# alibaba/unified-audio

Measured on AMD Instinct MI355X. Metric: audio-seconds/sec H-Codec encode+decode @16kHz b=32, higher is better.
Workload: dtype f32

## Files before the change

include/quarkaudio.h:

```cpp
#ifndef QUARKAUDIO_H_
#define QUARKAUDIO_H_

#include <stdint.h>

#ifdef __cplusplus
extern "C" {
#endif

#define QA_VERSION 103

typedef enum qa_status {
    QA_OK = 0,
    QA_ERR_INVALID = -1,
    QA_ERR_HIP = -2,
    QA_ERR_MISSING = -3,
    QA_ERR_UNSUPPORTED = -4
} qa_status;

typedef struct qa_tensor {
    const char* name;
    const float* data;
    int64_t numel;
} qa_tensor;

// ... 114 lines not shown
    int32_t post_act;
    int32_t in_rep;
} qa_conv_args;
int qa_conv1d_cl(const qa_conv_args* args, void* stream);

int qa_weight_planes(const float* w, int64_t n, void* planes, void* stream);
int qa_weight_planes_attach(const float* w, int64_t n, const void* planes);
int qa_weight_planes_detach(const float* w);
int64_t qa_weight_planes_bytes(void);
int64_t qa_weight_plane_offset(int64_t index, int32_t plane);

int qa_sconv_geometry(int64_t L, int32_t ksize, int32_t stride, int64_t* T_out, int32_t* pad_left, int32_t* pad_right);
int64_t qa_resolve_frame(int64_t r, int64_t L, int32_t max_pad, int32_t pad_mode);

int qa_profile_begin(void);
int qa_profile_end(double* out, int32_t n_out);
int qa_profile_begin_ex(int32_t mask);
int qa_profile_hbm_kinds(void);
const char* qa_profile_hbm_name(int32_t kind);
int qa_profile_end_hbm(double* out, int32_t n_out);
int qa_set_serial(int32_t on);

int qa_debug_lstm_stats(int32_t device, int64_t* out4);

int qa_knob_count(void);
int qa_knob_info(int32_t index, const char** name, int64_t* value, int64_t* default_value, const char** doc);
int qa_set_knob(const char* name, int64_t value);
int qa_get_knob(const char* name, int64_t* value);

typedef struct qa_ssl_spec {
    int32_t n_conv;
    int32_t conv_dim[8];
    int32_t conv_kernel[8];
    int32_t conv_stride[8];
    int32_t conv_bias;
    int32_t feat_norm_layer;
    int32_t hidden;
    int32_t n_layers;
    int32_t n_heads;
    int32_t intermediate;
    int32_t stable_layer_norm;
    int32_t pos_kernel;
    int32_t pos_groups;
    int32_t pad;
    int32_t n_select;
    int32_t select[32];
// ... 184 lines not shown
```

unified_audio_amd/_lib.py:

```python
from __future__ import annotations

import ctypes as C
import os
from typing import Optional

_HERE = os.path.dirname(os.path.abspath(__file__))
_LIB_NAME = "libquarkaudio_hip.so"
_lib: Optional[C.CDLL] = None


class QuarkAudioError(RuntimeError):

    def __init__(self, status: int, message: str):
        super().__init__(f"[qa_status {status}] {message}")
        self.status = status


class qa_tensor(C.Structure):
    _fields_ = [("name", C.c_char_p), ("data", C.c_void_p), ("numel", C.c_int64)]


class qa_hcodec_spec(C.Structure):
    _fields_ = [
        ("n_filters", C.c_int32), ("n_ratios", C.c_int32), ("ratios", C.c_int32 * 8), ("dimension", C.c_int32),
# ... 111 lines not shown
    "qa_hcodec_forward_adaptive": (C.c_int, [C.c_void_p, C.c_void_p, C.c_int64, C.c_int64, C.c_void_p, C.c_int64, C.c_int64,
                                             C.c_int64, C.c_int64, C.c_void_p, C.c_void_p, C.c_void_p, C.POINTER(C.c_int64),
                                             C.c_void_p]),
    "qa_hcodec_enable_taps": (C.c_int, [C.c_void_p, C.c_int]),
    "qa_hcodec_tap": (C.c_int64, [C.c_void_p, C.c_char_p, C.c_void_p, C.c_int64, C.c_void_p]),
    "qa_rvq_search": (C.c_int, [C.c_void_p, C.c_int64, C.c_void_p, C.c_int32, C.c_int32, C.c_int32, C.c_void_p,
                                C.c_void_p, C.c_void_p]),
    "qa_rvq_lookup": (C.c_int, [C.c_void_p, C.c_int64, C.c_void_p, C.c_int32, C.c_int32, C.c_int32, C.c_void_p,
                                C.c_void_p]),
    "qa_conv1d_cl": (C.c_int, [C.POINTER(qa_conv_args), C.c_void_p]),
    "qa_weight_planes": (C.c_int, [C.c_void_p, C.c_int64, C.c_void_p, C.c_void_p]),
    "qa_weight_planes_attach": (C.c_int, [C.c_void_p, C.c_int64, C.c_void_p]),
    "qa_weight_planes_detach": (C.c_int, [C.c_void_p]),
    "qa_weight_planes_bytes": (C.c_int64, []),
    "qa_weight_plane_offset": (C.c_int64, [C.c_int64, C.c_int32]),
    "qa_sconv_geometry": (C.c_int, [C.c_int64, C.c_int32, C.c_int32, C.POINTER(C.c_int64), C.POINTER(C.c_int32), C.POINTER(C.c_int32)]),
    "qa_resolve_frame": (C.c_int64, [C.c_int64, C.c_int64, C.c_int32, C.c_int32]),
    "qa_profile_begin": (C.c_int, []),
    "qa_profile_end": (C.c_int, [C.POINTER(C.c_double), C.c_int32]),
    "qa_profile_begin_ex": (C.c_int, [C.c_int32]),
    "qa_profile_hbm_kinds": (C.c_int, []),
    "qa_profile_hbm_name": (C.c_char_p, [C.c_int32]),
    "qa_debug_lstm_stats": (C.c_int, [C.c_int32, C.POINTER(C.c_int64)]),
    "qa_profile_end_hbm": (C.c_int, [C.POINTER(C.c_double), C.c_int32]),
    "qa_set_serial": (C.c_int, [C.c_int32]),
    "qa_knob_count": (C.c_int, []),
    "qa_knob_info": (C.c_int, [C.c_int32, C.POINTER(C.c_char_p), C.POINTER(C.c_int64), C.POINTER(C.c_int64), C.POINTER(C.c_char_p)]),
    "qa_set_knob": (C.c_int, [C.c_char_p, C.c_int64]),
    "qa_get_knob": (C.c_int, [C.c_char_p, C.POINTER(C.c_int64)]),
    "qa_mimi_create": (C.c_int, [C.POINTER(C.c_void_p), C.POINTER(qa_mimi_spec), C.POINTER(qa_tensor), C.c_int64, C.c_char_p, C.c_int]),
    "qa_mimi_destroy": (None, [C.c_void_p]),
    "qa_mimi_forward": (C.c_int, [C.c_void_p, C.c_void_p, C.c_int64, C.c_int64, C.c_void_p, C.c_void_p]),
    "qa_mimi_stream_begin": (C.c_int, [C.c_void_p, C.c_int64]),
    "qa_mimi_stream_step": (C.c_int, [C.c_void_p, C.c_void_p, C.c_int64, C.c_void_p, C.c_void_p]),
    "qa_mimi_stream_reset": (C.c_int, [C.c_void_p]),
    "qa_mimi_stream_end": (C.c_int, [C.c_void_p]),
    "qa_mimi_stream_offset": (C.c_int64, [C.c_void_p]),
    "qa_ssl_create": (C.c_int, [C.POINTER(C.c_void_p), C.POINTER(qa_ssl_spec), C.POINTER(qa_tensor), C.c_int64, C.c_int]),
    "qa_ssl_destroy": (None, [C.c_void_p]),
    "qa_ssl_frames": (C.c_int64, [C.c_void_p, C.c_int64]),
    "qa_ssl_forward": (C.c_int, [C.c_void_p, C.c_void_p, C.c_int64, C.c_int64, C.c_void_p, C.c_void_p]),
    "qa_bicodec_create": (C.c_int, [C.POINTER(C.c_void_p), C.POINTER(qa_bicodec_spec), C.POINTER(qa_tensor), C.c_int64, C.c_int]),
    "qa_bicodec_destroy": (None, [C.c_void_p]),
    "qa_bicodec_hop": (C.c_int64, [C.c_void_p]),
    "qa_bicodec_detokenize": (C.c_int, [C.c_void_p, C.c_void_p, C.c_void_p, C.c_int64, C.c_int64, C.c_void_p, C.c_void_p]),
    "qa_bicodec_enable_taps": (C.c_int, [C.c_void_p, C.c_int]),
# ... 119 lines not shown
```

unified_audio_amd/csrc/attention.hip:

```cpp
#include "kernels.h"

#ifdef QA_ATT_TIMING
__device__ unsigned long long g_qa_att_timing[8];
#define QA_ATT_TICK(i)                                      \
    {                                                       \
        const long long now_ = __builtin_readcyclecounter(); \
        tacc[i] += now_ - tlast;                            \
        tlast = now_;                                       \
    }
extern "C" int qa_debug_att_timing(unsigned long long* out, int reset) {
    if (out && hipMemcpyFromSymbol(out, HIP_SYMBOL(g_qa_att_timing), sizeof(g_qa_att_timing)) != hipSuccess) return -1;
    if (reset) {
        unsigned long long z[8] = {0};
        if (hipMemcpyToSymbol(HIP_SYMBOL(g_qa_att_timing), z, sizeof(z)) != hipSuccess) return -1;
    }
    return 0;
}
#else
#define QA_ATT_TICK(i)
#endif

namespace qa {

typedef float f32x16 __attribute__((ext_vector_type(16)));
// ... 183 lines not shown
    if (lane == 0) {
        for (int i = 0; i < 4; ++i) atomicAdd(&g_qa_att_timing[i], (unsigned long long)tacc[i]);
        atomicAdd(&g_qa_att_timing[4], (unsigned long long)(tlast - tbegin));
        atomicAdd(&g_qa_att_timing[5], 1ULL);
        atomicAdd(&g_qa_att_timing[6], (unsigned long long)n_done);
    }
#endif

    if (qi < n_q) {
        const float inv = l_run > 0.f ? 1.f / l_run : 0.f;
        float* op = out + ((long long)b * n_q + qi) * ldo + head * HD + 4 * hh;
#pragma unroll
        for (int t = 0; t < DT; ++t)
#pragma unroll
            for (int c = 0; c < 4; ++c) {
                float4 w;
                w.x = o[t][4 * c + 0] * inv; w.y = o[t][4 * c + 1] * inv;
                w.z = o[t][4 * c + 2] * inv; w.w = o[t][4 * c + 3] * inv;
                *reinterpret_cast<float4*>(op + 32 * t + 8 * c) = w;
            }
    }
}

int launch_attention(const float* q, long long ldq, const float* k, const float* v, long long ldkv, float* out,
                     long long ldo, int B, int n_q, int n_keys, long long kv_batch_stride, int H, int hd, float scale,
                     int causal, hipStream_t s, const float* gate, const float* relbias, int R, int context, int q_pos0,
                     int ring_end, const unsigned char* kvalid) {
    QA_REQUIRE(n_q > 0 && n_keys > 0 && (!causal || ring_end > 0 || n_keys >= n_q), "attention: n_q=%d n_keys=%d", n_q, n_keys);
    QA_REQUIRE(context >= 0 && (context == 0 || causal) && (ring_end <= 0 || (causal && context > 0 && !gate)),
               "attention: a context window needs causal=1; the ring mode needs causal=1 and context > 0");
    QA_REQUIRE((ldq % 4) == 0 && (ldkv % 4) == 0 && (ldo % 4) == 0, "attention: strides must be multiples of 4");
    QA_REQUIRE((gate == nullptr) == (relbias == nullptr) && (!gate || (R >= 0 && !causal && n_q == n_keys)),
               "attention: gate and relbias come together, for non-causal self-attention");
    QA_REQUIRE(!kvalid || (!gate && !causal && n_q == n_keys), "attention: the key-padding mask is for non-causal self-attention without bias");
    dim3 grid((unsigned)ceil_div(n_q, 128), H, B);
    const int dbg = (int)knob(K_ATT_DEBUG);
#define QA_ATT(HD)                                                                                                          \
    if (kvalid)                                                                                                              \
        hipLaunchKernelGGL((attention_kernel<HD, false, true>), grid, dim3(256), 0, s, q, ldq, k, v, ldkv, kv_batch_stride, out, ldo, n_q, \
                           n_keys, scale, causal, nullptr, nullptr, 0, context, q_pos0, ring_end, dbg, kvalid);                 \
    else if (gate)                                                                                                                \
        hipLaunchKernelGGL((attention_kernel<HD, true>), grid, dim3(256), 0, s, q, ldq, k, v, ldkv, kv_batch_stride, out, ldo, n_q, \
                           n_keys, scale, causal, gate, relbias, R, context, q_pos0, ring_end, dbg, nullptr);                           \
    else                                                                                                                     \
        hipLaunchKernelGGL((attention_kernel<HD, false>), grid, dim3(256), 0, s, q, ldq, k, v, ldkv, kv_batch_stride, out, ldo, n_q, \
                           n_keys, scale, causal, nullptr, nullptr, 0, context, q_pos0, ring_end, dbg, nullptr)
    switch (hd) {
        case 32: QA_ATT(32); break;
        case 64: QA_ATT(64); break;
        case 96: QA_ATT(96); break;
        case 128: QA_ATT(128); break;
        default: qa::set_error("attention: head_dim=%d unsupported (32/64/96/128)", hd); return QA_ERR_UNSUPPORTED;
    }
#undef QA_ATT
    QA_LAUNCH_CHECK();
    return QA_OK;
}

}

extern "C" int qa_debug_attention(const float* q, long long ldq, const float* k, const float* v, long long ldkv, float* out, long long ldo,
                                  int B, int n_q, int n_keys, long long kv_bstride, int H, int hd, float scale, int causal, void* stream) {
    return qa::launch_attention(q, ldq, k, v, ldkv, out, ldo, B, n_q, n_keys, kv_bstride, H, hd, scale, causal,
                                static_cast<hipStream_t>(stream));
}

extern "C" int qa_debug_attention_ex(const float* q, long long ldq, const float* k, const float* v, long long ldkv, float* out,
                                     long long ldo, int B, int n_q, int n_keys, long long kv_bstride, int H, int hd, float scale,
                                     int causal, const float* gate, const float* relbias, int R, int context, int q_pos0, int ring_end,
                                     void* stream) {
    return qa::launch_attention(q, ldq, k, v, ldkv, out, ldo, B, n_q, n_keys, kv_bstride, H, hd, scale, causal,
                                static_cast<hipStream_t>(stream), gate, relbias, R, context, q_pos0, ring_end);
}
```

unified_audio_amd/csrc/host_util.h:

```cpp
#pragma once
#include <algorithm>
#include <cmath>
#include <cstring>
#include <string>
#include <unordered_map>
#include <utility>
#include <vector>

#include "kernels.h"
#include "split_planes.h"

namespace qa {

class HostTable {
   public:
    HostTable(const qa_tensor* t, int64_t n) {
        for (int64_t i = 0; i < n; ++i)
            if (t[i].name && t[i].data) map_[t[i].name] = &t[i];
    }
    const float* get(const std::string& name, int64_t numel) const {
        auto it = map_.find(name);
        if (it == map_.end()) {
            set_error("weight table: missing tensor '%s'", name.c_str());
            return nullptr;
// ... 98 lines not shown
    }
    int ensure(size_t bytes) {
        if (bytes <= cap) return QA_OK;
        if (ptr) QA_HIP(hipFree(ptr));
        ptr = nullptr;
        cap = 0;
        const size_t grown = bytes + bytes / 8;
        QA_HIP(hipMalloc(reinterpret_cast<void**>(&ptr), grown));
        cap = grown;
        return QA_OK;
    }
};

struct Tap {
    const float* ptr;
    int64_t numel;
};

struct Ctx {
    Arena arena;
    hipStream_t stream = nullptr;
    bool dry = false;
    bool gemm_fp32 = false;
    bool capture = false;
    std::unordered_map<std::string, Tap> taps;
    void tap(const std::string& name, const float* p, int64_t n) {
        if (!capture) return;
        float* copy = arena.alloc<float>((size_t)n);
        arena.pin();
        if (dry) return;
        (void)hipMemcpyAsync(copy, p, sizeof(float) * (size_t)n, hipMemcpyDeviceToDevice, stream);
        taps[name] = Tap{copy, n};
    }
};

struct ConvW {
    const float* w = nullptr;
    const float* b = nullptr;
    int N = 0, C_in = 0, ksize = 1;
    int algo_n = 0, algo_cin = 0;
};

inline int pad32(int c) { return (int)round_up(c, 32); }


enum { WN_NONE = 0, WN_FOLD = 1, WN_DETECT = 2 };
// ... 143 lines not shown
inline int layernorm_op(Ctx& c, const float* x, const float* w, const float* b, float* y, int64_t rows, int C, float eps) {
    return c.dry ? QA_OK : launch_layernorm(x, w, b, y, rows, C, eps, c.stream);
}
inline int rmsnorm_op(Ctx& c, const float* x, const float* w, float* y, int64_t rows, int C, float eps) {
    return c.dry ? QA_OK : launch_rmsnorm(x, w, y, rows, C, eps, c.stream);
}
inline int dwconv_op(Ctx& c, const float* x, const float* w_kc, const float* bias, const float* lnw, const float* lnb, float* y, int B,
                     int T, int C, int ksize, float eps, int pad_left = -1) {
    return c.dry ? QA_OK : launch_dwconv(x, w_kc, bias, lnw, lnb, y, B, T, C, ksize, eps, c.stream, pad_left);
}
inline int to_channel_last_op(Ctx& c, const float* x, long long sb, long long sc, long long st, float* y, int B, int C, int T) {
    return c.dry ? QA_OK : launch_to_channel_last(x, sb, sc, st, y, B, C, T, c.stream);
}
inline int rope_op(Ctx& c, float* qkv, const float* cos_sin, int B, int N, int H, int hd, long long ld, int pos0, int interleaved = 0,
                   int rot_heads = 0) {
    return c.dry ? QA_OK : launch_rope(qkv, cos_sin, B, N, H, hd, ld, pos0, c.stream, interleaved, rot_heads);
}
inline int attention_op(Ctx& c, const float* q, long long ldq, const float* k, const float* v, long long ldkv, float* out, long long ldo,
                        int B, int n_q, int n_keys, long long kv_batch_stride, int H, int hd, float scale, int causal,
                        const float* gate = nullptr, const float* relbias = nullptr, int R = 0, int context = 0, int q_pos0 = 0,
                        int ring_end = 0, const unsigned char* kvalid = nullptr) {
    if (c.dry) return QA_OK;
    return launch_attention(q, ldq, k, v, ldkv, out, ldo, B, n_q, n_keys, kv_batch_stride, H, hd, scale, causal, c.stream, gate, relbias, R,
                            context, q_pos0, ring_end, kvalid);
}


inline void arm(Ctx& c, Workspace& ws) {
    c.dry = false;
    c.taps.clear();
    c.arena.begin(ws.ptr, ws.cap);
}

struct NoPreGrow {
    int operator()(size_t) const { return QA_OK; }
};

template <typename G, typename P = NoPreGrow>
int plan(int device, hipStream_t stream, Ctx& c, Workspace& ws, G&& graph, P&& pre_grow = P()) {
    QA_HIP(hipSetDevice(device));
    c.stream = stream;
    c.dry = true;
    c.arena.begin(nullptr, 0);
    QA_TRY(graph());
    if (c.arena.peak() > ws.cap) QA_TRY(pre_grow(c.arena.peak()));
    QA_TRY(ws.ensure(c.arena.peak()));
    arm(c, ws);
// ... 77 lines not shown
```

unified_audio_amd/csrc/kernels.h:

```cpp
#pragma once
#include <algorithm>

#include "common.h"

namespace qa {

int launch_conv_in(const float* x, const float* w_kc, const float* bias, float* y, int B, int T, int Cout, int ksize,
                   hipStream_t s, int pad_left = -1);
bool seanet_front_supported(int C, int hid, int L);
int launch_seanet_front(const float* wav, const float* w0, const float* b0, const float* w3, const float* b3, const float* wsc,
                        const float* bsc, const float* wpw, const float* bpw, float* a, int B, int L, int C, int hid, int causal,
                        hipStream_t s);
int launch_rmsnorm(const float* x, const float* w, float* y, long long rows, int C, float eps, hipStream_t s);
int launch_layernorm(const float* x, const float* w, const float* b, float* y, long long rows, int C, float eps,
                     hipStream_t s);
int launch_dwconv(const float* x, const float* w_kc, const float* bias, const float* lnw, const float* lnb, float* y,
                  int B, int T, int C, int ksize, float eps, hipStream_t s, int pad_left = -1);
size_t groupnorm_scratch_bytes(int B, int T, int G);
int launch_groupnorm(const float* x, const float* w, const float* bias, float* y, double* scratch, int B, int T, int C,
                     int G, float eps, int swish, hipStream_t s);
int launch_rope(float* qkv, const float* cos_sin, int B, int N, int H, int hd, long long ld, int pos0, hipStream_t s,
                int interleaved = 0, int rot_heads = 0);
int launch_align(const float* sem, int B, int T, int D, float thr, int max_tokens, int* seg, int* start, int* len,
                 int* nseg, int* gmax, hipStream_t s);
// ... 3 lines not shown
                      int D, hipStream_t s);
int launch_codes_inject(const long long* idx, const int* len, long long* dst, int B, int T, int G, int Q, int K,
                        hipStream_t s);
int launch_adaptive_frames(const long long* codes, int B, int Q, int G, int K, int* totals, int* tmax, hipStream_t s);
int launch_token_lengths(const long long* codes, long long* out, int B, int Q, int G, int K, hipStream_t s);
int launch_deaggregate(const long long* codes, const long long* len_codes, long long* out, int B, int Q, int G, int T, int K,
                       hipStream_t s);
int launch_to_channel_last(const float* x, long long sb, long long sc, long long st, float* y, int B, int C, int T,
                           hipStream_t s);
int launch_codes_to_bqn(const long long* src, long long* dst, int B, int N, int Q, hipStream_t s);
int launch_codes_from_bqn(const long long* src, long long* dst, int B, int N, int Q, hipStream_t s);
int launch_stft_post(const float* ri, float* out, long long rows, int nb, int ldi, int ldo, hipStream_t s);
int launch_istft_spec(const float* y, float* S, long long rows, int nb, int ldy, int ldS, hipStream_t s);
int launch_istft_ola(const float* frames, const float* win, float* out, int B, int T, int n_fft, int hop, hipStream_t s);

int launch_codes_check(const long long* codes, long long n, long long limit, unsigned long long* bad, hipStream_t s);
int launch_codes_count(const long long* codes, long long n, long long lo, long long limit, unsigned long long* bad, hipStream_t s);
int launch_resample(const float* wav, const float* taps, float* out, int B, long long T, long long T_out, int orig, int nw, int width,
                    int ktaps, hipStream_t s);

int launch_attention(const float* q, long long ldq, const float* k, const float* v, long long ldkv, float* out,
                     long long ldo, int B, int n_q, int n_keys, long long kv_batch_stride, int H, int hd, float scale,
                     int causal, hipStream_t s, const float* gate = nullptr, const float* relbias = nullptr, int R = 0,
                     int context = 0, int q_pos0 = 0, int ring_end = 0, const unsigned char* kvalid = nullptr);
int launch_ring_append(const float* k, const float* v, long long ld, float* kc, float* vc, int B, int T, int d, int cap, int pos0,
                       hipStream_t s);

int launch_lstm(const float* xw, const float* w_hh_ug, float* h_out, float* c_state, int B, int T, int d,
                hipStream_t s, bool eager = false);
int lstm_call_begin(int dev, void** ticket);
int lstm_call_end(void* ticket, hipStream_t s, bool* failed);
void lstm_call_note_sync();
void lstm_force_per_step(bool on);

size_t rvq_scratch_floats(long long n_vec, int K, int D);
int launch_rvq_search(const float* x, long long n_vec, const float* codebooks, const float* e2, int Q, int K, int D,
                      long long* indices, float* quantized, long long ldq, float* scratch, hipStream_t s);
int launch_rvq_norms(const float* codebooks, float* e2, int QK, int D, hipStream_t s);
int launch_rvq_lookup(const long long* indices, long long n_vec, const float* codebooks, int Q, int K, int D, float* out,
                      long long ldo, hipStream_t s);

int launch_assemble_prompt(float* x, const float* task_vec, const float* enroll_sos, const float* enroll_emb,
                           const float* mix_sos, const float* mix_emb, int B, int Ne, int Nm, int d, hipStream_t s);
int launch_skinny_gemm(const float* x, long long ldx, const float* w, const float* bias, const float* gate, long long ldg,
                       const float* res, long long ldr, float* y, long long ldy, int M, int N, int K, int act, hipStream_t s,
                       float rms_eps, int dual);
int launch_rope_kv(float* qkv, const float* cs, float* kc, float* vc, int B, int n, int H, int hd, int pos0, int max_len,
// ... 52 lines not shown
```

unified_audio_amd/csrc/knobs.h:

```cpp
#pragma once
#include <cstdint>

namespace qa {

#define QA_KNOB_TABLE(X)                                                                                                           \
    X(SERIAL, "QA_SERIAL", 0, "1: no internal stream concurrency (every kernel alone on the device; = qa_set_serial)")           \
    X(GEMM_CFG, "QA_GEMM_CFG", -1, "force the conv_gemm tile: 0 = 128x32, 1 = 128x64, 2 = 128x128, 3 = 64x128, 4 = 64x64, 5 = 256x128 (LINEAR layers; else 128x128) (-1: cost model)")             \
    X(GEMM_256, "QA_GEMM_256", 0, "r06 experiment: 256x128 block tile (4 waves, 4x2 accumulators each) for LINEAR layers with M >= 8000 and N >= 1024; value = its efficiency relative to 128x128 in 1/1000 for the cost model (0: never chosen; QA_GEMM_CFG=5 forces it)") \
    X(GEMM_BK16, "QA_GEMM_BK16", 1 << 30, "largest K that takes the BK = 16 K-chunk variant")                                     \
    X(GEMM_BK16_MIN_TILES, "QA_GEMM_BK16_MIN_TILES", 384, "fewest tiles of a launch that take BK = 16")                          \
    X(GEMM_MATH, "QA_GEMM_MATH", 1, "conv_gemm arithmetic: 1 = split-6 (operands split into three bf16 planes, six v_mfma_f32_32x32x16_bf16 per 16-wide k group, fp32 accumulation), 0 = the fp32 chain (v_mfma_f32_32x32x2_f32)") \
    X(GEMM_PRESPLIT, "QA_GEMM_PRESPLIT", 1, "split-6 weights from a pre-split image: a weight store builds the three bf16 planes of all its weights once, at load (6 bytes per weight beside the fp32 blob; not built when 0 at load time), and conv_gemm's 128-column tiles copy them into LDS instead of splitting the weight tile in the K loop (narrower tiles keep the in-loop split); 0 at launch = ignore the image and split in the loop; same bits either way") \
    X(GEMM_LINEAR, "QA_GEMM_LINEAR", 1, "table-free K loop for ksize-1 layers")                                                  \
    X(GEMM_XCD, "QA_GEMM_XCD", 1, "XCD-aware tile order")                                                                        \
    X(GEMM_PANEL, "QA_GEMM_PANEL", 8, "conv_gemm tile order: column panels of this many tiles, row tiles fastest inside a panel (0: column tiles fastest over the whole row; 8: +4 % on N >= 4096 shapes, +1.2 % on H-Codec 2.0)") \
    X(ATT_DEBUG, "QA_ATT_DEBUG", 0, "attention_kernel debug bits: 1 always rescale, 2 extra barrier per tile, 4 wait for the prefetch at once, 8 no wave-uniform tile skip, 16 mask every tile") \
    X(SEANET_FUSED, "QA_SEANET_FUSED", 1, "fused conv0 + first SEANet residual block")                                           \
    X(MIMI_ROPE_WINDOW, "QA_MIMI_ROPE_WINDOW", 8192, "mimi streaming: positions covered by the RoPE table before the rolling window takes over (tests shrink it)") \
    X(LSTM_GRAPH, "QA_LSTM_GRAPH", 1, "replay the T step launches of an LSTM call from a cached hipGraph")                       \
    X(LSTM_PERSISTENT, "QA_LSTM_PERSISTENT", -1, "persistent recurrence kernel: -1 auto (d >= 1536), 0 off, 1 on for every supported width") \
    X(LSTM_XCD, "QA_LSTM_XCD", 1, "XCD-local LSTM recurrence for d = 512 / 768 (one launch, W_hh in the registers of every XCD's 32 CUs, sequences dealt to the XCDs, 32-member step barrier per XCD): 0 off (the per-step kernels), 1 agent-scope hand-off forms, 2 XCD-local forms (h stores that stay in the XCD's L2; H-Codec 1.0: 42.7 against 43.3 ms)") \
    X(LSTM_TEAM, "QA_LSTM_TEAM", 1, "team recurrence for d = 1024 (one launch: 4 teams of 64 workgroups, W_hh resident in registers, 8 sequences per team, agent-scope hand-offs; H-Codec 1.5 decoder: 134.1 -> 128.3 ms per step, profiles/r04_lstm_team_ab.txt): 0 = the per-step kernels") \
    X(LSTM_SPIN_LIMIT, "QA_LSTM_SPIN_LIMIT", 1 << 21, "persistent recurrence: polls of a barrier word before the barrier is declared broken") \
    X(LSTM_FAULT, "QA_LSTM_FAULT", 0, "1 (tests): the persistent kernel's barrier waits for a workgroup that does not exist, like a starved launch") \
    X(LM_GRAPH, "QA_LM_GRAPH", 0, "1: replay one captured decode step per token")                                                \
    X(LM_MLP_FUSED, "QA_LM_MLP_FUSED", 1, "decode step: gate/up + SwiGLU + down of 16 activation columns per workgroup in one launch emitting K-slice partials, summed by a reduce launch (0: separate gate/up and down launches)") \
    X(LM_PF, "QA_LM_PF", 7, "decode step: cross-launch L2 weight prefetch planes (bit mask; lm_decode.h PfArgs): 1 qkv launch -> o_proj weights, 2 o_proj launch -> fused-MLP weights, 4 MLP launch -> next layer's qkv weights (last layer: the head slice), 8 head launch -> layer 0 qkv weights") \
    X(LM_ROWSPLIT, "QA_LM_ROWSPLIT", 3, "decode step at 9 .. 16 sequences: two 8-row groups instead of one 16-row group in the qkv launch (bit 1) and the fused-MLP launch (bit 2)") \
    X(LM_CHAINS, "QA_LM_CHAINS", 0, "generate: number of concurrent chains on internal streams (0: ceil(B / 64) - one chain serves up to 64 sequences, two row groups of 32 per launch; a count that would put more than 64 sequences into a chain is raised)") \
    X(LM_SCORE_ROWS, "QA_LM_SCORE_ROWS", 4096, "qa_lm_score: target rows per output_head launch (the logits buffer holds this many rows of the full vocabulary; any value gives the same bits)")

enum Knob {
#define QA_KNOB_ENUM(id, name, def, doc) K_##id,
    QA_KNOB_TABLE(QA_KNOB_ENUM)
#undef QA_KNOB_ENUM
        K_COUNT
};

long long knob(Knob k);
// ... 4 lines not shown
```

unified_audio_amd/csrc/lm.cpp:

```cpp
#include <memory>

#include <cstdlib>

#include "host_util.h"
#include "lm_decode.h"

using namespace qa;

namespace {
struct LMLayer {
    ConvW qkv, o, gate, up, down;
    const float* qkv_dec = nullptr;
    const float* gu_dec = nullptr;
    const float* down_dec = nullptr;
};
constexpr int LM_MAX_POS = 4096;
constexpr int LM_MAX_CHAINS = 16;
}

struct StepGraph {
    hipGraphExec_t exec = nullptr;
    hipGraph_t graph = nullptr;
    uint64_t key = 0;
    void reset() {
// ... 581 lines not shown

static int lm_generate_impl(qa_lm* lm, int32_t task, const float* enroll_feats, int64_t n_enroll, const float* mix_feats,
                            int64_t n_mix, int64_t B, int32_t global_length, int32_t semantic_length, const SampleCfg& sc,
                            int64_t* global_ids, int64_t* semantic_ids, void* stream, bool cond_mode = false, const float* cond = nullptr,
                            int64_t Tc = 0) {
    const char* fn = cond_mode ? "qa_lm_generate_cond" : "qa_lm_generate";
    if (!lm || (!cond_mode && !mix_feats) || !global_ids || !semantic_ids) {
        set_error("%s: null argument", fn);
        return QA_ERR_INVALID;
    }
    QA_REQUIRE(cond_mode || (task >= 0 && task < lm->spec.num_tasks), "%s: task %d out of range (KeyError in the reference)", fn, task);
    QA_REQUIRE(B > 0 && (cond_mode || n_mix > 0) && global_length >= 0 && semantic_length >= 0, "%s: bad shape", fn);
    QA_REQUIRE(!cond_mode || (Tc >= 0 && Tc < LM_MAX_POS && (cond != nullptr) == (Tc > 0) && global_length + semantic_length > 0),
               "qa_lm_generate_cond: cond_embeds [B, T, hidden] with T > 0, or NULL with T = 0 (got T = %lld); at least one step", (long long)Tc);
    QA_REQUIRE(!enroll_feats || n_enroll > 0, "%s: enrollment given with no frames", fn);
    QA_REQUIRE(sc.temperature > 0.f && sc.temperature <= 1.0f, "%s: temperature must be in (0, 1] (llm.py:278)", fn);
    QA_REQUIRE(sc.top_k >= 0 && sc.top_p > 0.f, "%s: bad top_k / top_p", fn);
    QA_HIP(hipSetDevice(lm->device));
    if (sc.do_sample) QA_TRY(lm_sample_prepare());
    lm->tap_n[0] = lm->tap_n[1] = -1;
    if (lm->taps) QA_TRY(ensure_taps(lm, B, global_length, semantic_length, stream));
    Ctx& c = lm->ctx;
    c.gemm_fp32 = true;
    auto graph = [&] {
        return generate_graph(lm, c, task, enroll_feats, (int)n_enroll, mix_feats, (int)n_mix, (int)B, global_length, semantic_length,
                              (long long*)global_ids, (long long*)semantic_ids, sc, cond_mode, cond, (int)Tc);
    };
    QA_TRY(plan(lm->device, static_cast<hipStream_t>(stream), c, lm->ws, graph, [&](size_t bytes) -> int {
        hipStreamCaptureStatus cs = hipStreamCaptureStatusNone;
        if (hipStreamIsCapturing(c.stream, &cs) != hipSuccess) (void)hipGetLastError();
        QA_REQUIRE(cs != hipStreamCaptureStatusActive,
                   "qa_lm_generate under a stream capture needs %zu bytes of workspace, the handle holds %zu: make one call of the same shape outside "
                   "the capture first (with QA_LM_CHAINS=1 for batches above 32: a capturing caller gets the single-chain launches)",
                   bytes, lm->ws.cap);
        return grow_step_buffer(lm, lm->ws, bytes);
    }));
    int st = graph();
    if (st != QA_OK) {
        c.stream = static_cast<hipStream_t>(stream);
        for (hipStream_t cs : lm->chain_streams) (void)hipStreamSynchronize(cs);
    } else if (lm->taps) {
        lm->tap_n[0] = B * (int64_t)(global_length + (cond_mode ? 0 : 1)) * lm->spec.global_size;
        lm->tap_n[1] = B * (int64_t)semantic_length * lm->spec.semantic_size;
    }
    return st;
}
// ... 31 lines not shown
    QA_REQUIRE(!enroll_feats || n_enroll > 0, "%s: enrollment given with no frames", fn);
    QA_REQUIRE(label_smoothing >= 0.0 && label_smoothing <= 1.0, "%s: label_smoothing %g outside [0, 1]", fn, label_smoothing);
    QA_REQUIRE(n_mix <= LM_MAX_POS && n_enroll <= LM_MAX_POS && B <= (1 << 24), "%s: bad shape", fn);
    QA_HIP(hipSetDevice(lm->device));
    hipStream_t s = static_cast<hipStream_t>(stream);
    hipStreamCaptureStatus cs = hipStreamCaptureStatusNone;
    if (hipStreamIsCapturing(s, &cs) != hipSuccess) (void)hipGetLastError();
    const bool capturing = cs == hipStreamCaptureStatusActive;
    ScoreArgs a{cond_mode, cond, (int)Tc, task, enroll_feats ? (int)n_enroll : 0, (int)n_mix, (int)B, global_length, semantic_length, enroll_feats, mix_feats,
                reinterpret_cast<const long long*>(global_ids), reinterpret_cast<const long long*>(semantic_ids), label_smoothing, loss_per_seq,
                reinterpret_cast<long long*>(correct_per_seq), loss, acc};
    const int Lt = global_length + semantic_length + 2 - (cond_mode ? 1 : 0);
    lm->score_tap_n = -1;
    float* tap = nullptr;
    if (lm->taps) {
        QA_REQUIRE(!capturing, "qa_lm_score: taps (a test hook) are not supported under a stream capture");
        const size_t bytes = sizeof(float) * (size_t)B * Lt * vocab_of(lm->spec);
        if (bytes > lm->score_tap.cap) QA_HIP(hipDeviceSynchronize());
        QA_TRY(lm->score_tap.ensure(bytes));
        tap = reinterpret_cast<float*>(lm->score_tap.ptr);
    }
    Ctx c;
    c.gemm_fp32 = true;
    auto graph = [&] { return score_graph(lm, c, a, tap); };
    QA_TRY(plan(lm->device, s, c, lm->score_ws, graph, [&](size_t bytes) -> int {
        QA_REQUIRE(!capturing, "qa_lm_score under a stream capture needs %zu bytes of workspace, the handle holds %zu: make one call of the "
                   "same shape outside the capture first", bytes, lm->score_ws.cap);
        QA_HIP(hipDeviceSynchronize());
        return QA_OK;
    }));
    QA_TRY(graph());
    if (tap) lm->score_tap_n = (int64_t)B * Lt * vocab_of(lm->spec);
    return QA_OK;
}

int qa_lm_score(qa_lm* lm, int32_t task, const float* enroll_feats, int64_t n_enroll, const float* mix_feats, int64_t n_mix, int64_t B,
                const int64_t* global_ids, int32_t global_length, const int64_t* semantic_ids, int32_t semantic_length, double label_smoothing,
                float* loss_per_seq, int64_t* correct_per_seq, float* loss, float* acc, void* stream) {
    return lm_score_impl(lm, task, enroll_feats, n_enroll, mix_feats, n_mix, B, global_ids, global_length, semantic_ids, semantic_length,
                         label_smoothing, loss_per_seq, correct_per_seq, loss, acc, stream, false, nullptr, 0);
}

int qa_lm_score_cond(qa_lm* lm, const float* cond_embeds, int64_t T, int64_t B, const int64_t* global_ids, int32_t global_length,
                     const int64_t* semantic_ids, int32_t semantic_length, double label_smoothing, float* loss_per_seq,
                     int64_t* correct_per_seq, float* loss, float* acc, void* stream) {
    return lm_score_impl(lm, 0, nullptr, 0, nullptr, 0, B, global_ids, global_length, semantic_ids, semantic_length, label_smoothing,
// ... 79 lines not shown
```

Baseline: 3080.

## Add split-6 bf16 MFMA attention kernel emulating fp32 via three bf16 planes

Adds an attention kernel that splits Q, K, V and the softmax probabilities into three bf16 planes each and computes both products with six v_mfma_f32_32x32x16_bf16 per 16-wide k group, accumulating in fp32. This replaces the fp32 MFMA chain (32x32x2_f32), aiming at the higher bf16 matrix throughput. It is on by default through a new knob, and the LM paths force the old fp32 kernel. The cost is extra split arithmetic, three times the LDS footprint for K and V, and slightly different rounding. Debug counters and test hooks are also added.

```diff
diff --git a/include/quarkaudio.h b/include/quarkaudio.h
--- a/include/quarkaudio.h
+++ b/include/quarkaudio.h
@@ -160,6 +160,7 @@
 int qa_set_serial(int32_t on);
 
 int qa_debug_lstm_stats(int32_t device, int64_t* out4);
+int qa_debug_att_stats(int64_t* out2);
 
 int qa_knob_count(void);
 int qa_knob_info(int32_t index, const char** name, int64_t* value, int64_t* default_value, const char** doc);
diff --git a/unified_audio_amd/_lib.py b/unified_audio_amd/_lib.py
--- a/unified_audio_amd/_lib.py
+++ b/unified_audio_amd/_lib.py
@@ -157,6 +157,7 @@
     "qa_profile_hbm_kinds": (C.c_int, []),
     "qa_profile_hbm_name": (C.c_char_p, [C.c_int32]),
     "qa_debug_lstm_stats": (C.c_int, [C.c_int32, C.POINTER(C.c_int64)]),
+    "qa_debug_att_stats": (C.c_int, [C.POINTER(C.c_int64)]),
     "qa_profile_end_hbm": (C.c_int, [C.POINTER(C.c_double), C.c_int32]),
     "qa_set_serial": (C.c_int, [C.c_int32]),
     "qa_knob_count": (C.c_int, []),
diff --git a/unified_audio_amd/csrc/attention.hip b/unified_audio_amd/csrc/attention.hip
--- a/unified_audio_amd/csrc/attention.hip
+++ b/unified_audio_amd/csrc/attention.hip
@@ -1,4 +1,7 @@
 #include "kernels.h"
+#include "split_planes.h"
+
+#include <atomic>
 
 #ifdef QA_ATT_TIMING
 __device__ unsigned long long g_qa_att_timing[8];
@@ -229,10 +232,292 @@
     }
 }
 
+typedef __bf16 bf16x8 __attribute__((ext_vector_type(8)));
+typedef short s16x4 __attribute__((ext_vector_type(4)));
+typedef short s16x8 __attribute__((ext_vector_type(8)));
+
+__device__ __forceinline__ void split4_unit(const f32x4 x, u32x2& ph, u32x2& pm, u32x2& pl) {
+#pragma unroll
+    for (int i = 0; i < 2; ++i) {
+        const float a = x[2 * i], b = x[2 * i + 1];
+        const unsigned h = rne_bf16x2(a, b);
+        const float ra = a - __builtin_bit_cast(float, h << 16), rb = b - __builtin_bit_cast(float, h & 0xffff0000u);
+        const unsigned m = rne_bf16x2(ra, rb);
+        ph[i] = h;
+        pm[i] = m;
+        pl[i] = rne_bf16x2(ra - __builtin_bit_cast(float, m << 16), rb - __builtin_bit_cast(float, m & 0xffff0000u));
+    }
+}
+__device__ __forceinline__ bf16x8 frag8(const u32x2 lo, const u32x2 hi) {
+    const u32x4 t = {lo[0], lo[1], hi[0], hi[1]};
+    return __builtin_bit_cast(bf16x8, t);
+}
+
+template <int HD, bool BIAS, bool KMASK = false>
+__global__ __launch_bounds__(256, (HD <= 64 ? 3 : 2)) void attention_split_kernel(const float* __restrict__ q, long long ldq,
+                                                              const float* __restrict__ k, const float* __restrict__ v,
+                                                              long long ldkv, long long kv_bstride, float* __restrict__ out,
+                                                              long long ldo, int n_q, int n_keys, float scale, int causal,
+                                                              const float* __restrict__ gate, const float* __restrict__ relbias, int R,
+                                                              int context, int q_pos0, int ring_end, int dbg_arg,
+                                                              const unsigned char* __restrict__ kvalid) {
+#if defined(QA_ATT_DBG) && QA_ATT_DBG == 0
+    constexpr int dbg = 0;
+    (void)dbg_arg;
+#else
+    const int dbg = dbg_arg;
+#endif
+    constexpr int DT = HD / 32;
+    constexpr int NKG = HD / 16;
+    constexpr int KS = HD * 2 + 16;
+    constexpr int VS = (HD % 64 == 0) ? HD * 2 + 64 : HD * 2;
+    constexpr int KPLANE = 32 * KS, VPLANE = 32 * VS;
+    static_assert(VS % 256 == 64 || VS % 256 == 192, "V rows must be 16 banks apart (mod 64)");
+    __shared__ __attribute__((aligned(16))) char sK[3 * KPLANE];
+    __shared__ __attribute__((aligned(16))) char sV[3 * VPLANE];
+
+    const int tid = threadIdx.x, lane = tid & 63, wave = __builtin_amdgcn_readfirstlane(tid >> 6);
+    const int ql = lane & 31, hh = lane >> 5;
+    const int b = blockIdx.z, head = blockIdx.y;
+    const int q_blk0 = blockIdx.x * 128;
+    const int qi = q_blk0 + wave * 32 + ql;
+    const int off = n_keys - n_q;
+    const int zpl = (dbg >> 5) & 7, zsel = (dbg >> 8) & 15;
+    const int zq = (zsel == 0 || (zsel & 1)) ? zpl : 0, zk = (zsel == 0 || (zsel & 2)) ? zpl : 0;
+    const int zv = (zsel == 0 || (zsel & 4)) ? zpl : 0, zp = (zsel == 0 || (zsel & 8)) ? zpl : 0;
+
+    constexpr float LOG2E = 1.4426950408889634f;
+    const float qs = scale * LOG2E;
+    bf16x8 qf[3][NKG];
+    {
+        const int qrow = qi < n_q ? qi : n_q - 1;
+        const float* qp = q + ((long long)b * n_q + qrow) * ldq + head * HD + 8 * hh;
+#pragma unroll
+        for (int g = 0; g < NKG; ++g) {
+            u32x2 p0[3], p1[3];
+            split4_rne(*reinterpret_cast<const f32x4*>(qp + 16 * g) * qs, p0[0], p0[1], p0[2]);
+            split4_rne(*reinterpret_cast<const f32x4*>(qp + 16 * g + 4) * qs, p1[0], p1[1], p1[2]);
+#pragma unroll
+            for (int pl = 0; pl < 3; ++pl) {
+                if (zq & (1 << pl)) p0[pl] = p1[pl] = u32x2{0u, 0u};
+                qf[pl][g] = frag8(p0[pl], p1[pl]);
+            }
+        }
+    }
+
+    float gate_q = 0.f;
+    const float* rb = nullptr;
+    if (BIAS) {
+        gate_q = LOG2E * gate[((long long)b * gridDim.y + head) * n_q + (qi < n_q ? qi : n_q - 1)];
+        rb = relbias + (long long)head * (2 * R + 1) + R;
+    }
+
+    f32x16 o[DT];
+#pragma unroll
+    for (int t = 0; t < DT; ++t)
+#pragma unroll
+        for (int r = 0; r < 16; ++r) o[t][r] = 0.f;
+    float m_run = -INFINITY, l_run = 0.f;
+
+    const float* kb = k + (long long)b * kv_bstride + head * HD;
+    const float* vb = v + (long long)b * kv_bstride + head * HD;
+
+    const bool ring = ring_end > 0;
+    const bool lin_causal = causal && !ring;
+    int last_key = n_keys - 1, first_key = 0;
+    if (lin_causal) {
+        const int q_last = min(q_blk0 + 127, n_q - 1);
+        last_key = min(last_key, q_last + off);
+        if (context > 0) first_key = max(0, q_blk0 + off - context + 1);
+    }
+    const int n_tiles = last_key / 32 + 1, kt0 = first_key / 32;
+    const int wave_last_key = lin_causal ? min(n_keys - 1, min(q_blk0 + wave * 32 + 31, n_q - 1) + off) : n_keys - 1;
+    const int wave_first_key = (lin_causal && context > 0) ? max(0, q_blk0 + wave * 32 + off - context + 1) : 0;
+    const int ring_idx = ring ? ring_end % n_keys : 0;
+
+    constexpr int NLD = HD / 32;
+    f32x4 kreg[NLD], vreg[NLD];
+    float mreg = 1.f;
+    const unsigned char* kvb = KMASK ? kvalid + (long long)b * n_keys : nullptr;
+    auto fetch = [&](int kt) {
+        if (KMASK) mreg = kvb[min(kt * 32 + (tid & 31), n_keys - 1)] ? 1.f : 0.f;
+#pragma unroll
+        for (int j = 0; j < NLD; ++j) {
+            const int i = tid + 256 * j;
+            const int row = i / (HD / 4), c4 = (i % (HD / 4)) * 4;
+            const int key = min(kt * 32 + row, n_keys - 1);
+            kreg[j] = *reinterpret_cast<const f32x4*>(kb + (long long)key * ldkv + c4);
+            vreg[j] = *reinterpret_cast<const f32x4*>(vb + (long long)key * ldkv + c4);
+        }
+    };
+    const char* kread = sK + ql * KS + 16 * hh;
+    const char* vread = sV + (4 * hh + ((lane & 15) >> 2)) * VS + 32 * ((lane >> 4) & 1) + 8 * (lane & 3);
+#ifdef QA_ATT_TIMING
+    long long tacc[4] = {0, 0, 0, 0};
+    long long tlast = __builtin_readcyclecounter();
+    const long long tbegin = tlast;
+    long long n_done = 0;
+#endif
+    fetch(kt0);
+    for (int kt = kt0; kt < n_tiles; ++kt) {
+        QA_ATT_TICK(3)
+        __syncthreads();
+#pragma unroll
+        for (int j = 0; j < NLD; ++j) {
+            const int i = tid + 256 * j;
+            const int row = i / (HD / 4), c4 = (i % (HD / 4)) * 4;
+            u32x2 pk[3], pv[3];
+            split4_rne(kreg[j], pk[0], pk[1], pk[2]);
+            split4_rne(vreg[j], pv[0], pv[1], pv[2]);
+            if (zk | zv) {
+#pragma unroll
+                for (int pl = 0; pl < 3; ++pl) {
+                    if (zk & (1 << pl)) pk[pl] = u32x2{0u, 0u};
+                    if (zv & (1 << pl)) pv[pl] = u32x2{0u, 0u};
+                }
+            }
+#pragma unroll
+            for (int pl = 0; pl < 3; ++pl) {
+                *reinterpret_cast<u32x2*>(sK + pl * KPLANE + row * KS + c4 * 2) = pk[pl];
+                *reinterpret_cast<u32x2*>(sV + pl * VPLANE + row * VS + c4 * 2) = pv[pl];
+            }
+            if (HD >= 96) __builtin_amdgcn_sched_barrier(0);
+        }
+        if (KMASK && tid < 32) *reinterpret_cast<float*>(sK + tid * KS + HD * 2) = mreg;
+        __syncthreads();
+        if (kt + 1 < n_tiles) fetch(kt + 1);
+        if (dbg & 4) asm volatile("s_waitcnt vmcnt(0)" ::: "memory");
+        if (dbg & 2) __syncthreads();
+        QA_ATT_TICK(0)
+        if (!(dbg & 8) && (kt * 32 > wave_last_key || kt * 32 + 31 < wave_first_key || q_blk0 + wave * 32 >= n_q)) continue;
+
+        constexpr int PA[6] = {0, 2, 1, 0, 1, 0}, PB[6] = {2, 0, 1, 1, 0, 0};
+        f32x16 s;
+#pragma unroll
+        for (int r = 0; r < 16; ++r) s[r] = 0.f;
+#pragma unroll
+        for (int g = 0; g < NKG; ++g) {
+            bf16x8 kf[3];
+#pragma unroll
+            for (int pl = 0; pl < 3; ++pl) kf[pl] = *reinterpret_cast<const bf16x8*>(kread + pl * KPLANE + 32 * g);
+#pragma unroll
+            for (int i = 0; i < 6; ++i) s = __builtin_amdgcn_mfma_f32_32x32x16_bf16(kf[PA[i]], qf[PB[i]][g], s, 0, 0, 0);
+            if (HD >= 96) __builtin_amdgcn_sched_barrier(0);
+        }
+        QA_ATT_TICK(1)
+        const int q_first = q_blk0 + wave * 32, q_last = q_first + 31;
+        const bool need_mask = KMASK || (dbg & 16) || ring || kt * 32 + 31 >= n_keys ||
+                               (lin_causal && (kt * 32 + 31 > q_first + off || (context > 0 && kt * 32 < q_last + off - context + 1)));
+        float tmax = -INFINITY;
+        if (BIAS || need_mask) {
+#pragma unroll
+            for (int r = 0; r < 16; ++r) {
+                const int key = kt * 32 + (r & 3) + 8 * (r >> 2) + 4 * hh;
+                bool ok = key < n_keys;
+                if (KMASK) ok = ok && *reinterpret_cast<const float*>(sK + ((r & 3) + 8 * (r >> 2) + 4 * hh) * KS + HD * 2) != 0.f;
+                if (ring) {
+                    const int delta = key - ring_idx;
+                    const int pos = key >= ring_end ? -1 : (delta <= 0 ? ring_end + delta : ring_end + delta - n_keys);
+                    const int dq = q_pos0 + qi - pos;
+                    ok = ok && pos >= 0 && dq >= 0 && dq < context;
+                } else if (causal) {
+                    ok = ok && key <= qi + off && (context <= 0 || qi + off - key < context);
+                }
+                float sc = s[r];
+                if (BIAS) sc += gate_q * rb[max(-R, min(R, key - qi))];
+                s[r] = ok ? sc : -INFINITY;
+            }
+        }
+#pragma unroll
+        for (int r = 0; r < 16; ++r) tmax = fmaxf(tmax, s[r]);
+        tmax = fmaxf(tmax, __shfl_xor(tmax, 32, 64));
+        const float m_new = fmaxf(m_run, tmax);
+        const float m_use = (m_new == -INFINITY) ? 0.f : m_new;
+        const float alpha = __builtin_amdgcn_exp2f(m_run - m_use);
+        float psum = 0.f;
+#pragma unroll
+        for (int r = 0; r < 16; ++r) {
+            s[r] = __builtin_amdgcn_exp2f(s[r] - m_use);
+            psum += s[r];
+        }
+        psum += __shfl_xor(psum, 32, 64);
+        l_run = l_run * alpha + psum;
+        m_run = m_new;
+        if ((dbg & 1) || __any(alpha != 1.f)) {
+#pragma unroll
+            for (int t = 0; t < DT; ++t)
+#pragma unroll
+                for (int r = 0; r < 16; ++r) o[t][r] *= alpha;
+        }
+        QA_ATT_TICK(2)
+#pragma unroll
+        for (int st = 0; st < 2; ++st) {
+            bf16x8 pf[3];
+            {
+                u32x2 p0[3], p1[3];
+                const f32x4 x0 = {s[8 * st + 0], s[8 * st + 1], s[8 * st + 2], s[8 * st + 3]};
+                const f32x4 x1 = {s[8 * st + 4], s[8 * st + 5], s[8 * st + 6], s[8 * st + 7]};
+                split4_unit(x0, p0[0], p0[1], p0[2]);
+                split4_unit(x1, p1[0], p1[1], p1[2]);
+                if (zp) {
+#pragma unroll
+                    for (int pl = 0; pl < 3; ++pl)
+                        if (zp & (1 << pl)) p0[pl] = p1[pl] = u32x2{0u, 0u};
+                }
+#pragma unroll
+                for (int pl = 0; pl < 3; ++pl) pf[pl] = frag8(p0[pl], p1[pl]);
+            }
+#pragma unroll
+            for (int t = 0; t < DT; ++t) {
+                bf16x8 vf[3];
+#pragma unroll
+                for (int pl = 0; pl < 3; ++pl) {
+                    const char* a = vread + pl * VPLANE + 16 * st * VS + 64 * t;
+                    const s16x4 lo = __builtin_amdgcn_ds_read_tr16_b64_v4i16((__attribute__((address_space(3))) s16x4*)(a));
+                    const s16x4 hi = __builtin_amdgcn_ds_read_tr16_b64_v4i16((__attribute__((address_space(3))) s16x4*)(a + 8 * VS));
+                    const s16x8 w = {lo[0], lo[1], lo[2], lo[3], hi[0], hi[1], hi[2], hi[3]};
+                    vf[pl] = __builtin_bit_cast(bf16x8, w);
+                }
+#pragma unroll
+                for (int i = 0; i < 6; ++i) o[t] = __builtin_amdgcn_mfma_f32_32x32x16_bf16(vf[PA[i]], pf[PB[i]], o[t], 0, 0, 0);
+                if (HD >= 96) __builtin_amdgcn_sched_barrier(0);
+            }
+        }
+#ifdef QA_ATT_TIMING
+        ++n_done;
+#endif
+    }
+#ifdef QA_ATT_TIMING
+    QA_ATT_TICK(3)
+    if (lane == 0) {
+        for (int i = 0; i < 4; ++i) atomicAdd(&g_qa_att_timing[i], (unsigned long long)tacc[i]);
+        atomicAdd(&g_qa_att_timing[4], (unsigned long long)(tlast - tbegin));
+        atomicAdd(&g_qa_att_timing[5], 1ULL);
+        atomicAdd(&g_qa_att_timing[6], (unsigned long long)n_done);
+    }
+#endif
+
+    if (qi < n_q) {
+        const float inv = l_run > 0.f ? 1.f / l_run : 0.f;
+        float* op = out + ((long long)b * n_q + qi) * ldo + head * HD + 4 * hh;
+#pragma unroll
+        for (int t = 0; t < DT; ++t)
+#pragma unroll
+            for (int c = 0; c < 4; ++c) {
+                float4 w;
+                w.x = o[t][4 * c + 0] * inv; w.y = o[t][4 * c + 1] * inv;
+                w.z = o[t][4 * c + 2] * inv; w.w = o[t][4 * c + 3] * inv;
+                *reinterpret_cast<float4*>(op + 32 * t + 8 * c) = w;
+            }
+    }
+}
+
+static std::atomic<long long> g_att_launches[2];
+
 int launch_attention(const float* q, long long ldq, const float* k, const float* v, long long ldkv, float* out,
                      long long ldo, int B, int n_q, int n_keys, long long kv_batch_stride, int H, int hd, float scale,
                      int causal, hipStream_t s, const float* gate, const float* relbias, int R, int context, int q_pos0,
-                     int ring_end, const unsigned char* kvalid) {
+                     int ring_end, const unsigned char* kvalid, bool math_fp32) {
     QA_REQUIRE(n_q > 0 && n_keys > 0 && (!causal || ring_end > 0 || n_keys >= n_q), "attention: n_q=%d n_keys=%d", n_q, n_keys);
     QA_REQUIRE(context >= 0 && (context == 0 || causal) && (ring_end <= 0 || (causal && context > 0 && !gate)),
                "attention: a context window needs causal=1; the ring mode needs causal=1 and context > 0");
@@ -242,16 +527,23 @@
     QA_REQUIRE(!kvalid || (!gate && !causal && n_q == n_keys), "attention: the key-padding mask is for non-causal self-attention without bias");
     dim3 grid((unsigned)ceil_div(n_q, 128), H, B);
     const int dbg = (int)knob(K_ATT_DEBUG);
-#define QA_ATT(HD)                                                                                                          \
+    const bool split = knob(K_ATT_MATH) != 0 && !math_fp32;
+#define QA_ATT_FORM(KERNEL, HD)                                                                                              \
     if (kvalid)                                                                                                              \
-        hipLaunchKernelGGL((attention_kernel<HD, false, true>), grid, dim3(256), 0, s, q, ldq, k, v, ldkv, kv_batch_stride, out, ldo, n_q, \
+        hipLaunchKernelGGL((KERNEL<HD, false, true>), grid, dim3(256), 0, s, q, ldq, k, v, ldkv, kv_batch_stride, out, ldo, n_q, \
                            n_keys, scale, causal, nullptr, nullptr, 0, context, q_pos0, ring_end, dbg, kvalid);                 \
     else if (gate)                                                                                                                \
-        hipLaunchKernelGGL((attention_kernel<HD, true>), grid, dim3(256), 0, s, q, ldq, k, v, ldkv, kv_batch_stride, out, ldo, n_q, \
+        hipLaunchKernelGGL((KERNEL<HD, true>), grid, dim3(256), 0, s, q, ldq, k, v, ldkv, kv_batch_stride, out, ldo, n_q, \
                            n_keys, scale, causal, gate, relbias, R, context, q_pos0, ring_end, dbg, nullptr);                           \
     else                                                                                                                     \
-        hipLaunchKernelGGL((attention_kernel<HD, false>), grid, dim3(256), 0, s, q, ldq, k, v, ldkv, kv_batch_stride, out, ldo, n_q, \
+        hipLaunchKernelGGL((KERNEL<HD, false>), grid, dim3(256), 0, s, q, ldq, k, v, ldkv, kv_batch_stride, out, ldo, n_q, \
                            n_keys, scale, causal, nullptr, nullptr, 0, context, q_pos0, ring_end, dbg, nullptr)
+#define QA_ATT(HD)                                   \
+    if (split) {                                     \
+        QA_ATT_FORM(attention_split_kernel, HD);     \
+    } else {                                         \
+        QA_ATT_FORM(attention_kernel, HD);           \
+    }
     switch (hd) {
         case 32: QA_ATT(32); break;
         case 64: QA_ATT(64); break;
@@ -259,11 +551,55 @@
         case 128: QA_ATT(128); break;
         default: qa::set_error("attention: head_dim=%d unsupported (32/64/96/128)", hd); return QA_ERR_UNSUPPORTED;
     }
+#undef QA_ATT_FORM
 #undef QA_ATT
     QA_LAUNCH_CHECK();
+    g_att_launches[split ? 1 : 0].fetch_add(1, std::memory_order_relaxed);
     return QA_OK;
 }
 
+}
+
+extern "C" int qa_debug_att_stats(int64_t* out2) {
+    if (!out2) {
+        qa::set_error("qa_debug_att_stats: bad argument");
+        return QA_ERR_INVALID;
+    }
+    for (int i = 0; i < 2; ++i) out2[i] = qa::g_att_launches[i].load(std::memory_order_relaxed);
+    return QA_OK;
+}
+
+namespace qa {
+__global__ void split_unit_check_kernel(const float* __restrict__ x, long long n4, unsigned long long* __restrict__ bad) {
+    const long long i = (long long)blockIdx.x * blockDim.x + threadIdx.x;
+    if (i >= n4) return;
+    const f32x4 v = *reinterpret_cast<const f32x4*>(x + 4 * i);
+    u32x2 a[3], b[3];
+    split4_rne(v, a[0], a[1], a[2]);
+    split4_unit(v, b[0], b[1], b[2]);
+    unsigned diff = 0;
+    for (int pl = 0; pl < 3; ++pl)
+        for (int e = 0; e < 2; ++e) diff += a[pl][e] != b[pl][e];
+    if (diff) atomicAdd(bad, 1ULL);
+}
+}
+
+extern "C" int qa_debug_att_split_unit(const float* x, long long n, unsigned long long* bad, void* stream) {
+    if (!x || !bad || n <= 0 || (n % 4) != 0) {
+        qa::set_error("qa_debug_att_split_unit: bad argument");
+        return QA_ERR_INVALID;
+    }
+    const long long n4 = n / 4;
+    hipLaunchKernelGGL(qa::split_unit_check_kernel, dim3((unsigned)((n4 + 255) / 256)), dim3(256), 0, static_cast<hipStream_t>(stream), x, n4, bad);
+    QA_LAUNCH_CHECK();
+    return QA_OK;
+}
+
+extern "C" int qa_debug_attention_kmask(const float* q, long long ldq, const float* k, const float* v, long long ldkv, float* out, long long ldo,
+                                        int B, int n_q, int n_keys, long long kv_bstride, int H, int hd, float scale,
+                                        const unsigned char* kvalid, void* stream) {
+    return qa::launch_attention(q, ldq, k, v, ldkv, out, ldo, B, n_q, n_keys, kv_bstride, H, hd, scale, 0, static_cast<hipStream_t>(stream),
+                                nullptr, nullptr, 0, 0, 0, 0, kvalid);
 }
 
 extern "C" int qa_debug_attention(const float* q, long long ldq, const float* k, const float* v, long long ldkv, float* out, long long ldo,
diff --git a/unified_audio_amd/csrc/host_util.h b/unified_audio_amd/csrc/host_util.h
--- a/unified_audio_amd/csrc/host_util.h
+++ b/unified_audio_amd/csrc/host_util.h
@@ -144,6 +144,7 @@
     hipStream_t stream = nullptr;
     bool dry = false;
     bool gemm_fp32 = false;
+    bool att_fp32 = false;
     bool capture = false;
     std::unordered_map<std::string, Tap> taps;
     void tap(const std::string& name, const float* p, int64_t n) {
@@ -333,7 +334,7 @@
                         int ring_end = 0, const unsigned char* kvalid = nullptr) {
     if (c.dry) return QA_OK;
     return launch_attention(q, ldq, k, v, ldkv, out, ldo, B, n_q, n_keys, kv_batch_stride, H, hd, scale, causal, c.stream, gate, relbias, R,
-                            context, q_pos0, ring_end, kvalid);
+                            context, q_pos0, ring_end, kvalid, c.att_fp32);
 }
 
 
diff --git a/unified_audio_amd/csrc/kernels.h b/unified_audio_amd/csrc/kernels.h
--- a/unified_audio_amd/csrc/kernels.h
+++ b/unified_audio_amd/csrc/kernels.h
@@ -49,7 +49,7 @@
 int launch_attention(const float* q, long long ldq, const float* k, const float* v, long long ldkv, float* out,
                      long long ldo, int B, int n_q, int n_keys, long long kv_batch_stride, int H, int hd, float scale,
                      int causal, hipStream_t s, const float* gate = nullptr, const float* relbias = nullptr, int R = 0,
-                     int context = 0, int q_pos0 = 0, int ring_end = 0, const unsigned char* kvalid = nullptr);
+                     int context = 0, int q_pos0 = 0, int ring_end = 0, const unsigned char* kvalid = nullptr, bool math_fp32 = false);
 int launch_ring_append(const float* k, const float* v, long long ld, float* kc, float* vc, int B, int T, int d, int cap, int pos0,
                        hipStream_t s);
 
diff --git a/unified_audio_amd/csrc/knobs.h b/unified_audio_amd/csrc/knobs.h
--- a/unified_audio_amd/csrc/knobs.h
+++ b/unified_audio_amd/csrc/knobs.h
@@ -14,7 +14,8 @@
     X(GEMM_LINEAR, "QA_GEMM_LINEAR", 1, "table-free K loop for ksize-1 layers")                                                  \
     X(GEMM_XCD, "QA_GEMM_XCD", 1, "XCD-aware tile order")                                                                        \
     X(GEMM_PANEL, "QA_GEMM_PANEL", 8, "conv_gemm tile order: column panels of this many tiles, row tiles fastest inside a panel (0: column tiles fastest over the whole row; 8: +4 % on N >= 4096 shapes, +1.2 % on H-Codec 2.0)") \
-    X(ATT_DEBUG, "QA_ATT_DEBUG", 0, "attention_kernel debug bits: 1 always rescale, 2 extra barrier per tile, 4 wait for the prefetch at once, 8 no wave-uniform tile skip, 16 mask every tile") \
+    X(ATT_MATH, "QA_ATT_MATH", 1, "attention arithmetic: 1 = split-6 (Q, K, V and the probabilities as three bf16 planes, six v_mfma_f32_32x32x16_bf16 per 16-wide k group, fp32 accumulation), 0 = the fp32 chain (v_mfma_f32_32x32x2_f32); the UniSE LM keeps the fp32 chain either way") \
+    X(ATT_DEBUG, "QA_ATT_DEBUG", 0, "attention_kernel debug bits: 1 always rescale, 2 extra barrier per tile, 4 wait for the prefetch at once, 8 no wave-uniform tile skip, 16 mask every tile; split-6 only (tests): 32 / 64 / 128 zero the h / m / l plane of the operands selected by 256 Q, 512 K, 1024 V, 2048 P (none of the four: all)") \
     X(SEANET_FUSED, "QA_SEANET_FUSED", 1, "fused conv0 + first SEANet residual block")                                           \
     X(MIMI_ROPE_WINDOW, "QA_MIMI_ROPE_WINDOW", 8192, "mimi streaming: positions covered by the RoPE table before the rolling window takes over (tests shrink it)") \
     X(LSTM_GRAPH, "QA_LSTM_GRAPH", 1, "replay the T step launches of an LSTM call from a cached hipGraph")                       \
diff --git a/unified_audio_amd/csrc/lm.cpp b/unified_audio_amd/csrc/lm.cpp
--- a/unified_audio_amd/csrc/lm.cpp
+++ b/unified_audio_amd/csrc/lm.cpp
@@ -627,6 +627,7 @@
     if (lm->taps) QA_TRY(ensure_taps(lm, B, global_length, semantic_length, stream));
     Ctx& c = lm->ctx;
     c.gemm_fp32 = true;
+    c.att_fp32 = true;
     auto graph = [&] {
         return generate_graph(lm, c, task, enroll_feats, (int)n_enroll, mix_feats, (int)n_mix, (int)B, global_length, semantic_length,
                               (long long*)global_ids, (long long*)semantic_ids, sc, cond_mode, cond, (int)Tc);
@@ -704,6 +705,7 @@
     }
     Ctx c;
     c.gemm_fp32 = true;
+    c.att_fp32 = true;
     auto graph = [&] { return score_graph(lm, c, a, tap); };
     QA_TRY(plan(lm->device, s, c, lm->score_ws, graph, [&](size_t bytes) -> int {
         QA_REQUIRE(!capturing, "qa_lm_score under a stream capture needs %zu bytes of workspace, the handle holds %zu: make one call of the "
```

Result: faster. 3141 (median of 6 runs) (+2.0%).
